# andvg3/LipVQ-VAE

Measured on AMD Instinct MI355X. Metric: actions tokenized/sec (encode+quantize) at B=4096 T=128 K=1024, 1/2/4/8 GPU, higher is better.
Workload: dtype f32

## Files before the change

lipvq-vae_amd/csrc/lipvq_fused.hip:

```cpp
#include <string.h>
#include <atomic>

#include "lipvq_mlp.h"
#include "lipvq_screen.h"

#define FUSED_WAVES 8
#define FUSED_THREADS (FUSED_WAVES * 64)
#define FUSED_HIST_MAX 2048
#define LQ_RING8_TC 1
#define LQ_RING8_NB 3
#define LQ_RING13_NB 3
constexpr int fused_ring_tc(int S) { return (S <= 2) ? 4 : (S <= 4) ? 2 : (S == 8) ? LQ_RING8_TC : 1; }
constexpr int fused_ring_nb(int S) { return (S <= 4) ? 4 : (S == 8) ? LQ_RING8_NB : LQ_RING13_NB; }
#define LQ_COARSE_TC_WIDE 2
constexpr int fused_ring_tc_coarse(int S) { return S == 8 ? LQ_COARSE_TC_WIDE * fused_ring_tc(S) : fused_ring_tc(S); }

struct Gelu2 {
    lq_v2f x, t, u, s;
    __device__ __forceinline__ void stage0(float a, float b) {
        x = (lq_v2f){a, b};
        t = x * x;
        u = lq_fma2(t, lq_bc2(0.11111111111111111111f), lq_bc2(-1.0f));
        s = lq_fma2(lq_bc2(0.00012666420661844313f), u, lq_bc2(-0.00043783686123788357f));
        s = lq_fma2(s, u, lq_bc2(0.0008924771682359278f));
// ... 55 lines not shown
    const float* x;
    const float* packed;
    const unsigned char* packed16;
    const unsigned char* prep;
    const float* cb;
    int64_t* idx;
    float* zq;
    unsigned long long* usage;
    float* ze_out;
    int* amb_count;
    int* amb_list;
    const float* w2q;
    float* pre0;
    float* pre1;
    float* pre2;
    int64_t N;
    int A, D, K;
    float gamma;
    int coarse;
    int inplace;
    int defer_ze;
    int nt_ze;
    int ze_ring;
    int keepz;
};

template <int S, bool FAST, bool TRAIN, int WAVES, bool COARSE = false, bool VQ = false, bool KEEPZ = false>
__device__ __forceinline__ void tokenize_body(const TokArgs& a) {
    static_assert(!(FAST && TRAIN), "training uses the parity arithmetic");
    static_assert(!VQ || !FAST, "the ReLU instance: parity arithmetic");
    static_assert(!KEEPZ || (S <= 4 && !FAST && !TRAIN && !COARSE && !VQ), "z_e kept in registers: the narrow parity instances, decided in place");
    constexpr int THREADS = WAVES * 64;
    constexpr int TCF = COARSE ? fused_ring_tc_coarse(S) : fused_ring_tc(S), NBF = fused_ring_nb(S);
    using RingCfg = ScreenCfg<S, TCF, COARSE>;
    constexpr size_t SLAB_STRIDE = ScreenCfg<S, fused_ring_tc(S), false>::STAGE_BYTES;
    constexpr int T0 = 2, T1 = 4, T2 = (S + 1) / 2;
    constexpr int S1 = 16 * T0, S2 = 16 * T1;
    constexpr bool STREAM2 = !FAST && S >= LQ_STREAM2_MIN_S;
    static_assert(!FAST || (S % 2 == 0 && S <= 8), "fast mode: D in {32, 64, 128}");
    extern __shared__ __attribute__((aligned(16))) unsigned char lds[];
#ifdef LQ_STAMPS
    const long long st_top = __builtin_amdgcn_s_memtime();
    const long long st_top_rt = (long long)__builtin_amdgcn_s_memrealtime();
#endif

    const PackedLayout PL = packed_layout(a.A, 32 * T0, 32 * T1, 16 * S);
    const PrepLayout L = prep_layout(a.K, a.D);
    const int S0 = PL.S0;
    const int S0q = (S0 + 3) / 4;
    const int S0h = (a.A + 15) / 16;
    float* w_P0 = reinterpret_cast<float*>(lds);
    float* w_B0 = w_P0 + (FAST ? T0 * S0h * 256 : T0 * S0q * 256);
    float* w_P1 = w_B0 + 32 * T0;
    float* w_B1 = w_P1 + (FAST ? T1 * (2 * T0) * 256 : T1 * (S1 / 4) * 256);
    float* w_P2 = w_B1 + 32 * T1;
    float* w_B2 = w_P2 + (FAST ? T2 * (2 * T1) * 256 : STREAM2 ? 0 : T2 * (S2 / 4) * 256);
    float* w_mu = w_B2 + 32 * T2;
    unsigned char* stage0 = reinterpret_cast<unsigned char*>(w_mu + 16 * S);
    constexpr size_t RING_OWN = (size_t)NBF * RingCfg::STAGE_BYTES + 1024, RING_FINE = lq_ring_bytes<S, fused_ring_tc(S), NBF>();
    constexpr size_t STAGES_BYTES = RING_OWN > RING_FINE ? RING_OWN : RING_FINE;
    static_assert(STAGES_BYTES >= (size_t)WAVES * LQ_DECIDE_BYTES, "the decision's per-wave transposes live in the stage ring");
    constexpr size_t WSLICE = (STAGES_BYTES >= (size_t)WAVES * 8192) ? 8192 : LQ_DECIDE_BYTES;
    static_assert(LQ_DECIDE_BYTES >= 4096 && WSLICE >= LQ_DECIDE_BYTES, "a slice holds the transposes and four staged KiB");
    static_assert(!KEEPZ || WSLICE >= LQ_DECIDE_BYTES + 64 * S, "KEEPZ: one z_e row behind the decision scratch");
    unsigned* hist = reinterpret_cast<unsigned*>(stage0 + ((STAGES_BYTES + 63) & ~(size_t)63));
    const bool use_hist = a.usage && fused_hist_fits<S, FAST>(a.A, a.K);

    const int tid = threadIdx.x, lane = tid & 63;
    const int wave = __builtin_amdgcn_readfirstlane(tid >> 6);
    const int ln = lane & 31, h = lane >> 5;

    const unsigned* hdr = reinterpret_cast<const unsigned*>(a.prep);
    const unsigned char* tiles = a.prep + (COARSE ? L.o_tiles_hi : L.o_tiles);
    const size_t tile_bytes = COARSE ? L.tile_bytes_hi : L.tile_bytes;
    const int sz = lq_scale_exp(1.0f + __uint_as_float(hdr[4]));
    const float fz = lq_pow2f(sz);
    const float fown = lq_pow2f(sz + (int)hdr[3]);
    const float tiny2 = (float)(16 * S) * lq_pow2f(-10 - 2 * sz);
    const int64_t nblk = (a.N + WAVES * 32 - 1) / (WAVES * 32);
    constexpr int XPF = 8;
    const bool x_pref = !FAST && a.A <= 2 * XPF;
    float xq[XPF];
    constexpr int LANE_W_MIN_S = 8;
    auto load_x = [&](int64_t blk_, float (&out)[XPF]) {
        int64_t r_ = (blk_ * WAVES + wave) * 32 + ln;
        r_ = r_ < a.N ? r_ : a.N - 1;
        const int64_t last = a.N * a.A - 1;
        int h_x = h;
        if constexpr (S >= LANE_W_MIN_S) asm volatile("" : "+v"(h_x));
#pragma unroll
        for (int q = 0; q < XPF; ++q) {
            const int k = 2 * q + h_x;
            int64_t i_ = r_ * a.A + k;
            i_ = i_ < last ? i_ : last;
            const float v = a.x[i_];
            out[q] = (k < a.A) ? v : 0.0f;
        }
    };
    if (x_pref) load_x(blockIdx.x, xq);
    lq_ws_begin(a.amb_count);
    {
        static_assert(32 * T1 <= THREADS && 32 * T2 <= THREADS && 16 * S <= THREADS, "one element per thread");
        const float* mu = reinterpret_cast<const float*>(a.prep + L.o_mu);
        auto bias_src = [&](size_t o, int n) { const int i = tid < n ? tid : n - 1; return a.packed[o + 32 * (i >> 5) + 2 * (i & 15) + ((i >> 4) & 1)]; };
        const float vb0 = bias_src(PL.oB0, 32 * T0), vb1 = bias_src(PL.oB1, 32 * T1), vb2 = bias_src(PL.oB2, 32 * T2);
        const float vmu = mu[tid < 16 * S ? tid : 16 * S - 1];
        if (FAST) {
            const float* src = reinterpret_cast<const float*>(a.packed16);
            const int n0 = T0 * S0h * 256, n1 = T1 * (2 * T0) * 256, n2 = T2 * (2 * T1) * 256;
            auto copy16 = [&](float* dst, const float* from, int nfl) {
                const float4* s4 = reinterpret_cast<const float4*>(from);
                float4* d4 = reinterpret_cast<float4*>(dst);
                const int nv = nfl / 4;
                for (int v0 = tid; v0 < nv; v0 += 4 * THREADS) {
                    float4 r[4];
#pragma unroll
                    for (int q = 0; q < 4; ++q) { const int v = v0 + q * THREADS; r[q] = s4[v < nv ? v : nv - 1]; }
#pragma unroll
                    for (int q = 0; q < 4; ++q) { const int v = v0 + q * THREADS; if (v < nv) d4[v] = r[q]; }
                }
            };
            copy16(w_P0, src, n0);
            copy16(w_P1, src + n0, n1);
            copy16(w_P2, src + n0 + n1, n2);
        } else {
            constexpr int NV1 = T1 * (S1 / 4) * 64, NV2 = STREAM2 ? 0 : T2 * (S2 / 4) * 64;
            constexpr int R1 = (NV1 + THREADS - 1) / THREADS, R2 = (NV2 + THREADS - 1) / THREADS;
            const float* P0 = a.packed + PL.oP0;
            const float* P1 = a.packed + PL.oP1;
            const float* P2 = a.packed + PL.oP2;
            float4 r1[R1], r2[R2 > 0 ? R2 : 1];
#pragma unroll
            for (int it = 0; it < R1; ++it) {
                int v = tid + it * THREADS;
                v = v < NV1 ? v : NV1 - 1;
                const float* src = P1 + ((size_t)(v >> 6) * 4) * 64 + (v & 63);
                r1[it] = make_float4(src[0], src[64], src[128], src[192]);
            }
#pragma unroll
            for (int it = 0; it < R2; ++it) {
                int v = tid + it * THREADS;
                v = v < NV2 ? v : NV2 - 1;
                const float* src = P2 + ((size_t)(v >> 6) * 4) * 64 + (v & 63);
                r2[it] = make_float4(src[0], src[64], src[128], src[192]);
            }
            const int NV0 = T0 * S0q * 64;
            auto p0_entry = [&](int v0, float (&e)[4]) {
                const int l = v0 & 63, sq = (v0 >> 6) % S0q, t = (v0 >> 6) / S0q;
#pragma unroll
                for (int q = 0; q < 4; ++q) {
                    const int s = 4 * sq + q;
                    const float v = P0[((size_t)t * S0 + (s < S0 ? s : S0 - 1)) * 64 + l];
                    e[q] = (s < S0) ? v : 0.0f;
                }
            };
            float e0[4];
            p0_entry(tid < NV0 ? tid : NV0 - 1, e0);
            if (tid < NV0) *reinterpret_cast<float4*>(w_P0 + (size_t)tid * 4) = make_float4(e0[0], e0[1], e0[2], e0[3]);
            for (int v0 = tid + THREADS; v0 < NV0; v0 += THREADS) {
                float e[4];
                p0_entry(v0, e);
                *reinterpret_cast<float4*>(w_P0 + (size_t)v0 * 4) = make_float4(e[0], e[1], e[2], e[3]);
            }
#pragma unroll
            for (int it = 0; it < R1; ++it) {
                const int v = tid + it * THREADS;
                if (v < NV1) *reinterpret_cast<float4*>(w_P1 + (size_t)v * 4) = r1[it];
            }
#pragma unroll
            for (int it = 0; it < R2; ++it) {
                const int v = tid + it * THREADS;
                if (v < NV2) *reinterpret_cast<float4*>(w_P2 + (size_t)v * 4) = r2[it];
            }
        }
        if (tid < 32 * T0) w_B0[tid] = vb0;
        if (tid < 32 * T1) w_B1[tid] = vb1;
        if (tid < 32 * T2) w_B2[tid] = vb2;
        if (tid < 16 * S) w_mu[tid] = vmu;
        if (use_hist)
            for (int i = tid; i < a.K; i += THREADS) hist[i] = 0u;
    }
// ... 60 lines not shown
                acc[r] = zv;
                const float v = zv - w_mu[32 * t + 2 * r + h_w];
                zt[t][r] = v;
                n2 = lq_fma(v, v, n2);
                amax = fmaxf(amax, lq_abs(v));
            }
          } else {
            if constexpr (!FAST) {
                lq_v2f chk = lq_bc2(0.0f);
#pragma unroll
                for (int r = 0; r < 16; r += 2) chk = lq_nonfinite_acc2((lq_v2f){acc[r], acc[r + 1]}, chk);
                if (__builtin_amdgcn_ballot_w64(!(chk.x == 0.0f && chk.y == 0.0f)) != 0ull) {
#pragma unroll
                    for (int r = 0; r < 16; ++r) acc[r] = lq_sigmoid(acc[r]);
                } else {
#pragma unroll
                    for (int r = 0; r < 16; r += 2) {
                        if (2 * t + (r >> 3) >= S) continue;
                        const lq_v2f z2 = lq_sigmoid2_finite((lq_v2f){acc[r], acc[r + 1]});
                        acc[r] = z2.x; acc[r + 1] = z2.y;
                    }
                }
            }
#pragma unroll
            for (int r = 0; r < 16; ++r) {
                if (2 * t + (r >> 3) >= S) continue;
                const float zv = FAST ? __builtin_amdgcn_rcpf(1.0f + __builtin_amdgcn_exp2f(acc[r] * -1.44269504088896341f)) : acc[r];
                acc[r] = zv;
                const float v = zv - w_mu[32 * t + 2 * r + h_w];
                n2 = lq_fma(v, v, n2);
                const float vs = v * fz;
                const _Float16 vh = (_Float16)vs;
                const float rs = vs - (float)vh;
                ah[2 * t + (r >> 3)][r & 7] = vh;
                al[2 * t + (r >> 3)][r & 7] = (_Float16)rs;
                if constexpr (COARSE) a2lo = lq_fma(rs, rs, a2lo);
            }
          }
            if constexpr (KEEPZ) {
                zkeep[t] = acc;
            } else if (a.ze_out) {
                if (DEFER_ZE && a.defer_ze && t == T2 - 1) zdef = acc;
                else store_ze_tile(row, t, acc);
            }
        };

        if constexpr (!FAST) {
            auto gelu_fixup = [&](f32x16& out, const f32x16& pre) {
                float mx = 0.0f;
#pragma unroll
                for (int r = 0; r < 16; r += 2) asm("v_max3_f32 %0, %1, |%2|, |%3|" : "=v"(mx) : "v"(mx), "v"(pre[r]), "v"(pre[r + 1]));
                if (__builtin_amdgcn_ballot_w64(!(mx * mx < 18.0f)) != 0ull) {
#pragma unroll
                    for (int r = 0; r < 16; ++r)
                        if (!(pre[r] * pre[r] < 18.0f)) out[r] = lq_gelu_tail(pre[r]);
                }
            };
            auto bias16 = [&](const float* wb, int t) {
                f32x16 b;
                const float4* p4 = reinterpret_cast<const float4*>(wb + (2 * t + h) * 16);
#pragma unroll
                for (int q = 0; q < 4; ++q) { const float4 v = p4[q]; b[4 * q] = v.x; b[4 * q + 1] = v.y; b[4 * q + 2] = v.z; b[4 * q + 3] = v.w; }
                return b;
            };
            f32x16 h0[T0];
            constexpr int NTRIP = (16 * S + 63) / 64;
            constexpr int GP = (STAGES_BYTES >= (size_t)WAVES * 8192) ? 8 : 4;
            constexpr int NROUND = NTRIP * (8 / GP);
            unsigned char* gstage = stage0 + (size_t)wave * WSLICE;
            const bool gnow = DEFER_GATHER && have_pend && a.zq;
            if (gnow) lq_gather_dma<GP>(gstage, a.cb, pend_k, pend_ok, pend_row0, a.N, a.D, lane, 0, 0);
            {
#pragma unroll
                for (int t = 0; t < T0; ++t) h0[t] = bias16(w_B0, t);
                if (x_pref) {
#pragma unroll
                    for (int sq = 0; sq < XPF / 4; ++sq) {
                        if (sq < S0q) {
                            float4 av[T0];
#pragma unroll
                            for (int t = 0; t < T0; ++t) av[t] = *reinterpret_cast<const float4*>(w_P0 + ((t * S0q + sq) * 64 + lane_w) * 4);
#pragma unroll
                            for (int q = 0; q < 4; ++q) {
                                const float bv = xq[4 * sq + q];
#pragma unroll
                                for (int t = 0; t < T0; ++t) {
                                    const float aq = q == 0 ? av[t].x : q == 1 ? av[t].y : q == 2 ? av[t].z : av[t].w;
                                    h0[t] = __builtin_amdgcn_mfma_f32_32x32x2f32(aq, bv, h0[t], 0, 0, 0);
                                }
                            }
                        }
                    }
                } else {
                    const float* xr = a.x + (size_t)rowc * a.A;
                    for (int sq = 0; sq < S0q; ++sq) {
                        float4 av[T0];
                        float bvv[4];
#pragma unroll
                        for (int t = 0; t < T0; ++t) av[t] = *reinterpret_cast<const float4*>(w_P0 + ((t * S0q + sq) * 64 + lane_w) * 4);
#pragma unroll
                        for (int q = 0; q < 4; ++q) {
                            const int k = 2 * (4 * sq + q) + h;
                            bvv[q] = (k < a.A) ? xr[k] : 0.0f;
                        }
#pragma unroll
                        for (int q = 0; q < 4; ++q)
#pragma unroll
                            for (int t = 0; t < T0; ++t) {
                                const float aq = q == 0 ? av[t].x : q == 1 ? av[t].y : q == 2 ? av[t].z : av[t].w;
                                h0[t] = __builtin_amdgcn_mfma_f32_32x32x2f32(aq, bvv[q], h0[t], 0, 0, 0);
                            }
                    }
                }
#pragma unroll
                for (int t = 0; t < T0; ++t) {
                    const f32x16 pre = h0[t];
                    if constexpr (TRAIN) lq_tile_store16(a.pre0, 32 * T0, row, row < a.N, t, h, pre, 32 * T0, true);
                    if constexpr (VQ) {
#pragma unroll
                        for (int r = 0; r < 16; ++r) h0[t][r] = pre[r] > 0.0f ? pre[r] : 0.0f;
                    } else {
#pragma unroll
                    for (int r = 0; r < 16; r += 2) {
                        const lq_v2f g2 = lq_gelu_poly2((lq_v2f){pre[r], pre[r + 1]});
                        h0[t][r] = g2.x; h0[t][r + 1] = g2.y;
                    }
                    gelu_fixup(h0[t], pre);
                    }
                }
            }
            if (gnow) {
#pragma unroll
                for (int rd = 0; rd < NROUND; ++rd) {
                    lq_wait_vmcnt<0>();
                    lq_gather_flush<GP>(gstage, a.zq, pend_ok, pend_row0, a.N, a.D, lane, rd / (8 / GP), GP * (rd % (8 / GP)));
                    if (rd + 1 < NROUND) {
                        asm volatile("s_waitcnt lgkmcnt(0)" ::: "memory");
                        lq_gather_dma<GP>(gstage, a.cb, pend_k, pend_ok, pend_row0, a.N, a.D, lane, (rd + 1) / (8 / GP),
                                          GP * ((rd + 1) % (8 / GP)));
                    }
                }
            }
            LQ_STAMP(0);
            f32x16 h1[T1];
            f32x16 pend;
            constexpr bool LUMPED = !VQ && !STREAM2;
            constexpr int G1 = S1 / 4, G2 = S2 / 4;
            auto wread = [&](int gidx) {
                if (STREAM2 && gidx >= T1 * G1) gidx = T1 * G1 - 1;
                return (gidx < T1 * G1) ? *reinterpret_cast<const float4*>(w_P1 + (gidx * 64 + lane_w) * 4)
                                        : *reinterpret_cast<const float4*>(w_P2 + ((gidx - T1 * G1) * 64 + lane_w) * 4);
            };
            auto slab_dma = [&](int t_, int buf_) {
                const unsigned char* src = reinterpret_cast<const unsigned char*>(a.w2q) + (size_t)t_ * (G2 * 1024);
                unsigned char* dst = stage0 + (size_t)buf_ * SLAB_STRIDE;
                unsigned lane16 = (unsigned)lane * 16u;
                asm volatile("" : "+v"(lane16));
#pragma unroll
                for (int j = 0; j < G2 * 1024 / 1024 / WAVES; ++j) {
                    const int off = (wave + j * WAVES) * 1024;
                    const unsigned long long gaddr = (unsigned long long)(uintptr_t)(src + off) + lane16;
                    const unsigned ldsaddr = __builtin_amdgcn_readfirstlane((unsigned)(uintptr_t)(dst + off));
                    unsigned m0_keep;
                    asm volatile("s_mov_b32 %0, m0\n\ts_mov_b32 m0, %2\n\ts_nop 0\n\tglobal_load_lds_dwordx4 %1, off\n\ts_mov_b32 m0, %0"
                                 : "=&s"(m0_keep) : "v"(gaddr), "s"(ldsaddr) : "memory");
                }
            };
// ... 104 lines not shown
                f16x8 bx;
#pragma unroll
                for (int j = 0; j < 8; ++j) {
                    const int k = 16 * s2 + 2 * j + h;
                    bx[j] = (_Float16)((k < a.A) ? xr[k] : 0.0f);
                }
#pragma unroll
                for (int t = 0; t < T0; ++t) {
                    const f16x8 av = *reinterpret_cast<const f16x8*>(wh0 + ((size_t)(t * S0h + s2) * 64 + lane) * 8);
                    h0[t] = __builtin_amdgcn_mfma_f32_32x32x16_f16(av, bx, h0[t], 0, 0, 0);
                }
            }
            f16x8 b0[2 * T0];
#pragma unroll
            for (int t = 0; t < T0; ++t)
#pragma unroll
                for (int r = 0; r < 16; ++r) b0[2 * t + (r >> 3)][r & 7] = (_Float16)lq_gelu(h0[t][r]);
            f16x8 b1[2 * T1];
#pragma unroll
            for (int t = 0; t < T1; ++t) {
                f32x16 acc;
#pragma unroll
                for (int r = 0; r < 16; ++r) acc[r] = w_B1[(2 * t + h) * 16 + r];
#pragma unroll
                for (int s2 = 0; s2 < 2 * T0; ++s2) {
                    const f16x8 av = *reinterpret_cast<const f16x8*>(wh1 + ((size_t)(t * (2 * T0) + s2) * 64 + lane) * 8);
                    acc = __builtin_amdgcn_mfma_f32_32x32x16_f16(av, b0[s2], acc, 0, 0, 0);
                }
#pragma unroll
                for (int r = 0; r < 16; ++r) b1[2 * t + (r >> 3)][r & 7] = (_Float16)lq_gelu(acc[r]);
            }
#pragma unroll
            for (int t = 0; t < T2; ++t) {
                f32x16 acc;
#pragma unroll
                for (int r = 0; r < 16; ++r) acc[r] = w_B2[(2 * t + h) * 16 + r];
#pragma unroll
                for (int s2 = 0; s2 < 2 * T1; ++s2) {
                    const f16x8 av = *reinterpret_cast<const f16x8*>(wh2 + ((size_t)(t * (2 * T1) + s2) * 64 + lane) * 8);
                    acc = __builtin_amdgcn_mfma_f32_32x32x16_f16(av, b1[s2], acc, 0, 0, 0);
                }
                finish_tile(t, acc);
            }
        }
        LQ_STAMP(2);
        n2 += __shfl_xor(n2, 32, 64);
        row_n2 = n2;
        row_fz = fz;
        row_fown = fown;
        if constexpr (VQ) {
            amax = fmaxf(amax, __shfl_xor(amax, 32, 64));
            const int szr = lq_scale_exp(amax);
            const float fzr = lq_pow2f(szr);
            row_fz = fzr;
            row_fown = lq_pow2f(szr + (int)hdr[3]);
#pragma unroll
            for (int t = 0; t < T2; ++t)
#pragma unroll
                for (int r = 0; r < 16; ++r) {
                    if (2 * t + (r >> 3) >= S) continue;
                    const float vs = zt[t][r] * fzr;
                    const _Float16 vh = (_Float16)vs;
                    const float rs = vs - (float)vh;
                    ah[2 * t + (r >> 3)][r & 7] = vh;
                    al[2 * t + (r >> 3)][r & 7] = (_Float16)rs;
                    if constexpr (COARSE) a2lo = lq_fma(rs, rs, a2lo);
                }
        }
        if constexpr (COARSE) a2lo += __shfl_xor(a2lo, 32, 64);
        row_a2 = a2lo;
      };
        encode();
        float frow[16];
        if constexpr (VQ) lq_row_factors(row_fown, lane, frow);
        else {
#pragma unroll
            for (int r = 0; r < 16; ++r) frow[r] = fown;
        }
        float m1[16], m2[16];
        int k1[16];
#pragma unroll
        for (int r = 0; r < 16; ++r) { m1[r] = INFINITY; m2[r] = INFINITY; k1[r] = 0; }
        LQ_STAMP(3);
        if (x_pref) load_x(blk + gridDim.x < nblk ? blk + gridDim.x : blk, xq);
        constexpr bool PACKF = S <= 4 || S > 8 || COARSE;
        const float zn = COARSE ? lq_coarse_zn(row_a2, row_n2, row_fz, row_fown, __uint_as_float(hdr[5])) : 0.0f;
        float znr[16];
        if constexpr (COARSE) lq_row_factors(zn, lane, znr);
        else {
#pragma unroll
            for (int r = 0; r < 16; ++r) znr[r] = 0.0f;
        }
        if constexpr (KEEPZ) {
            lq_screen_core<S, THREADS, TCF, NBF, PACKF, COARSE>(ah, al, tiles, L.ntiles, stage0, tid, frow, znr, m1, m2, k1);
        } else {
            const bool have_def = DEFER_ZE && a.defer_ze && a.ze_out != nullptr;
            const bool wave_def = __builtin_amdgcn_ballot_w64((blk * WAVES + wave) * 32 + ln < a.N) != 0ull;
            auto deferred_ze = [&]() { store_ze_tile((blk * WAVES + wave) * 32 + ln, T2 - 1, zdef); };
            lq_screen_core<S, THREADS, TCF, NBF, PACKF, COARSE, 4, decltype(deferred_ze)>(ah, al, tiles, L.ntiles, stage0, tid, frow, znr, m1, m2, k1, have_def, deferred_ze, wave_def);
        }
        LQ_STAMP(4);
        const unsigned keep_mask = PACKF ? ~((1u << lq_pack_bits(L.ntiles)) - 1u) : 0xffffffffu;
        unsigned char* scratch = stage0 + (size_t)wave * WSLICE;
        const int64_t row0 = (blk * WAVES + wave) * 32;
        const int64_t row = row0 + ln;
        int my_k;
        LqDecision dec;
        bool certified = lq_screen_decide<PACKF, COARSE>(m1, m2, k1, scratch, hdr, row_n2, row_fown, a.gamma, a.K, a.D, lane,
                                                         my_k, dec, PACKF ? lq_pow2f(lq_pack_bits(L.ntiles) - 23) : 0.0f, keep_mask,
                                                         zn, tiles, tile_bytes, ScreenCfg<S, TCF, COARSE>::FRAG_BYTES);
        const bool row_sane = VQ || row_n2 >= tiny2;
        certified = certified && row_sane;
        if constexpr (KEEPZ)
            certified = lq_screen_decide_inplace<PACKF, 2 * S, LIPVQ_DIST_NORM, T2>(
                dec, certified, row_sane, my_k, row0, row < a.N, a.amb_count, nullptr, a.cb, a.K, lane, keep_mask, scratch, zkeep);
        else if (!COARSE && a.inplace)
            certified = lq_screen_decide_inplace<PACKF, 2 * S, VQ ? LIPVQ_DIST_SQSUM : LIPVQ_DIST_NORM>(
                dec, certified, row_sane, my_k, row0 - ze_shift, row < a.N, a.amb_count, a.ze_out, a.cb, a.K, lane, keep_mask, scratch);
        else
            lq_screen_emit<PACKF>(dec, certified, row_sane, my_k, row, row < a.N, a.amb_count, a.amb_list, a.N, a.K, lane, keep_mask, scratch);
        if (h == 0 && row < a.N && certified) {
            a.idx[row] = (int64_t)my_k;
            if (use_hist) atomicAdd(&hist[my_k], 1u);
        }
        if (a.usage && !use_hist) lq_usage_add(a.usage, my_k, h == 0 && row < a.N && certified);
        if (DEFER_GATHER) { pend_k = my_k; pend_ok = certified; pend_row0 = row0; }
        else if (a.zq) lq_screen_gather(a.cb, a.zq, my_k, certified, row0, a.N, a.D, lane);
        if (DEFER_GATHER) have_pend = true;
        LQ_STAMP(5);
        LQ_STAMP(6);
    }
    if (DEFER_GATHER && have_pend && a.zq) lq_screen_gather(a.cb, a.zq, pend_k, pend_ok, pend_row0, a.N, a.D, lane);
#ifdef LQ_STAMPS
    if (lane == 0) {
        long long* dbg = LqWorkspace::from_lists(a.amb_list, a.N).stamps() + ((size_t)blockIdx.x * WAVES + wave) * 16;
        for (int i = 0; i < 7; ++i) dbg[i] = st_acc[i];
        dbg[7] = 0;
        dbg[8] = __builtin_amdgcn_s_memtime() - st_begin;
        dbg[9] = st_begin;
        dbg[10] = st_begin - st_top;
        dbg[11] = (long long)__builtin_amdgcn_s_memrealtime();
        dbg[12] = st_top_rt;
    }
#endif
    lq_ws_publish(a.amb_count);
    if (use_hist) {
        for (int i = tid; i < a.K; i += THREADS) {
            const unsigned c = hist[i];
            if (c) atomicAdd(&a.usage[i], (unsigned long long)c);
        }
    }
}

template <int S, bool FAST, bool TRAIN = false, bool COARSE = false, bool VQ = false, bool KEEPZ = false>
__global__ __launch_bounds__(FUSED_THREADS) void tokenize_kernel(TokArgs a) {
    tokenize_body<S, FAST, TRAIN, FUSED_WAVES, COARSE, VQ, KEEPZ>(a);
}
template <int S, bool FAST, bool TRAIN, bool COARSE = false, bool KEEPZ = false>
__global__ __launch_bounds__(256) __attribute__((amdgpu_waves_per_eu(1, 1))) void tokenize_kernel_w4(TokArgs a) {
    tokenize_body<S, FAST, TRAIN, 4, COARSE, false, KEEPZ>(a);
}

__global__ void mlp3_pack_f16_kernel(const float* __restrict__ W0, const float* __restrict__ W1, const float* __restrict__ W2,
                                     _Float16* __restrict__ out, int A, int J0, int J1, int D) {
    const int S0h = (A + 15) / 16, S1h = J0 / 16, S2h = J1 / 16;
    const int T0 = J0 / 32, T1 = J1 / 32, T2 = (D + 31) / 32;
    const size_t n0 = (size_t)T0 * S0h * 512, n1 = (size_t)T1 * S1h * 512, n2 = (size_t)T2 * S2h * 512;
    size_t g = (size_t)blockIdx.x * blockDim.x + threadIdx.x;
    if (g >= n0 + n1 + n2) return;
    const float* W;
    int K, J, Sh;
    size_t e = g;
    if (e < n0) { W = W0; K = A; J = J0; Sh = S0h; }
    else if (e < n0 + n1) { e -= n0; W = W1; K = J0; J = J1; Sh = S1h; }
    else { e -= n0 + n1; W = W2; K = J1; J = D; Sh = S2h; }
    const int j = (int)(e & 7), lane = (int)((e >> 3) & 63);
    const size_t ts = e >> 9;
    const int s = (int)(ts % Sh), t = (int)(ts / Sh);
    const int f = 32 * t + feat_of_tile_row(lane & 31);
    const int k = 16 * s + 2 * j + (lane >> 5);
    out[g] = (_Float16)((f < J && k < K) ? W[(size_t)f * K + k] : 0.0f);
}
// ... 293 lines not shown
```

lipvq-vae_amd/csrc/lipvq_screen.h:

```cpp
#ifndef LIPVQ_SCREEN_H_
#define LIPVQ_SCREEN_H_
#include <hip/hip_fp16.h>

#include <type_traits>

#include "lipvq_common.h"

typedef _Float16 f16x8 __attribute__((ext_vector_type(8)));

#define LIPVQ_SCREEN_GAMMA 3.814697265625e-06f
#define SCREEN_WAVES 8

struct PrepLayout {
    int S, Dpad, Kpad, ntiles;
    size_t o_hdr, o_mu, o_tiles, tile_bytes, total;
    size_t o_tiles_hi, tile_bytes_hi;
};

#define LIPVQ_SCREEN_GAMMA_WIDE 1.52587890625e-05f
#define LQ_SCREEN_NARROW_MAX_S 13

__host__ __device__ static inline int lq_screen_S(int D) {
    const int s = (D + 15) / 16;
    return D <= 0 ? 0 : s <= 2 ? 2 : s <= 4 ? 4 : s <= 8 ? 8 : s <= 13 ? 13 : s <= 16 ? 16 : s <= 24 ? 24 : s <= 32 ? 32 : 0;
// ... 22 lines not shown

__device__ __forceinline__ int lq_scale_exp(float maxabs) {
    const int e = (int)((__float_as_uint(maxabs) >> 23) & 0xff) - 127;
    int k = 13 - e;
    k = k < -60 ? -60 : k;
    k = k > 60 ? 60 : k;
    return (maxabs > 0.0f && maxabs < INFINITY) ? k : 0;
}
__device__ __forceinline__ float lq_pow2f(int k) { return __uint_as_float((unsigned)(k + 127) << 23); }

constexpr int screen_default_tc(int S) { return (S <= 2) ? 8 : (S <= 4) ? 4 : (S <= 8) ? 2 : 1; }

template <int S, int TC_ = screen_default_tc(S), bool COARSE = false>
struct ScreenCfg {
    static constexpr int FRAG_BYTES = COARSE ? S * 1024 : S * 2048;
    static constexpr int TILE_BYTES = FRAG_BYTES + 256;
    static constexpr int TC = TC_;
    static constexpr int STAGE_BYTES = TC * TILE_BYTES;
    static constexpr int STAGE_VEC = STAGE_BYTES / 16;
};

template <int S>
struct StandaloneScreen {
    static constexpr int TC = (S <= 2) ? 4 : (S <= 4) ? 2 : 1;
    static constexpr int NB = (S <= 8) ? 4 : 3;
    static constexpr bool PACK = S <= 4;
};

template <bool PACK>
__device__ __forceinline__ void lq_track_one(float v, int id, unsigned keep_mask, float& m1, float& m2, int& k1) {
    if constexpr (PACK) {
        float key;
        asm("v_and_or_b32 %0, %1, %2, %3" : "=v"(key) : "v"(v), "s"(keep_mask), "v"(id));
        m2 = __builtin_amdgcn_fmed3f(key, m1, m2);
        asm("v_min_f32 %0, %1, %2" : "=v"(m1) : "v"(key), "v"(m1));
    } else {
        const bool lt = v < m1;
        k1 = lt ? id : k1;
        m2 = __builtin_amdgcn_fmed3f(v, m1, m2);
        m1 = lt ? v : m1;
    }
}

__device__ __forceinline__ float lq_coarse_zn(float a2lo, float n2, float fz, float fown, float rho) {
    const float A = lq_sqrt(a2lo), B = lq_sqrt(n2) * fz;
    const float t = lq_fma(rho, lq_fma(3.0f, A, B), A);
    return t * (fown / fz) * 1.0009765625f;
}
template <int LO, int HI, bool PACK = false, bool COARSE = false>
__device__ __forceinline__ void lq_track_part(const f32x16& acc, float e2, float en, const float (&frow)[16], const float (&znr)[16],
                                              int id, unsigned keep_mask, float (&m1)[16], float (&m2)[16], int (&k1)[16]) {
#pragma unroll
    for (int r = LO; r < HI; ++r) {
        const float v = COARSE ? acc[r] : lq_fma(e2, frow[r], acc[r]);
        lq_track_one<PACK>(v, id, keep_mask, m1[r], m2[r], k1[r]);
    }
}

template <int S, bool PACK, bool COARSE = false>
__device__ __forceinline__ void lq_track_after_mfma(int j, const f32x16& acc, float e2, float en, const float (&frow)[16],
                                                    const float (&znr)[16], int id, unsigned keep_mask, float (&m1)[16],
                                                    float (&m2)[16], int (&k1)[16]) {
    constexpr int NM = COARSE ? S : 3 * S;
    const int lo = (16 * j) / NM, hi = (16 * (j + 1)) / NM;
#pragma unroll
    for (int r = 0; r < 16; ++r)
        if (r >= lo && r < hi) {
            const float v = COARSE ? acc[r] : lq_fma(e2, frow[r], acc[r]);
            lq_track_one<PACK>(v, id, keep_mask, m1[r], m2[r], k1[r]);
        }
}

template <int N>
__device__ __forceinline__ void lq_wait_vmcnt() {
    static_assert(N >= 0 && N < 64, "vmcnt immediate");
    asm volatile("s_waitcnt vmcnt(%0)" ::"n"(N) : "memory");
}
template <int S, int TC_, int NB>
constexpr size_t lq_ring_bytes() { return (size_t)NB * ScreenCfg<S, TC_>::STAGE_BYTES + 1024; }

__host__ __device__ static inline int lq_pack_bits(int ntiles) { int b = 1; while ((1 << b) < ntiles) ++b; return b; }

struct LqNoDeferred { __device__ __forceinline__ void operator()() const {} };
template <int S, int NT, int TC_ = screen_default_tc(S), int NB = 4, bool PACK = false, bool COARSE = false, int NDEF = 0,
          typename DEFERRED = LqNoDeferred>
__device__ __forceinline__ void lq_screen_core(const f16x8 (&ah)[S], const f16x8 (&al)[S],
                                               const unsigned char* __restrict__ tiles, int ntiles,
                                               unsigned char* stage0, int tid, const float (&frow)[16], const float (&znr)[16],
                                               float (&m1)[16], float (&m2)[16], int (&k1)[16],
                                               bool have_def = false, DEFERRED deferred = DEFERRED(), bool wave_def = true) {
    using C = ScreenCfg<S, TC_, COARSE>;
    static_assert(NB >= 3 && NB <= 4, "ring of 3 or 4 stage buffers");
    constexpr int NW = NT / 64;
    constexpr int CHUNKS = (C::STAGE_BYTES + 1023) / 1024;
    constexpr int CPW = (CHUNKS + NW - 1) / NW;
    constexpr int PD = NB - 1;
    constexpr int NSTEP = C::TC * S;
    constexpr int MID = (C::TC >= 2) ? (C::TC / 2) * S : S / 2;
    constexpr int FR = 2;
    constexpr int FD = FR - 1;
    constexpr int PERIOD = ((C::TC & 1) || (NSTEP % FR)) ? 2 : 1;
    static_assert(C::STAGE_BYTES >= 1024 && C::STAGE_BYTES % 16 == 0, "stage copies are whole KiB pieces");
    static_assert(NSTEP - FD >= MID, "next-stage fragments are read after the hand-over");
    static_assert(CPW * PD < 64, "vmcnt immediate");
    const int lane = tid & 63, ln = lane & 31;
    const int wave = __builtin_amdgcn_readfirstlane(tid >> 6);
    const int nstage = ntiles / C::TC;
    unsigned char* dummy = stage0 + (size_t)NB * C::STAGE_BYTES;
    typedef __attribute__((address_space(3))) void* lds_ptr_t;
    typedef const __attribute__((address_space(1))) void* glb_ptr_t;
    auto stage_dma = [&](int st, int buf) {
        const bool real = st < nstage;
        const unsigned char* src = tiles + (real ? (size_t)st * C::STAGE_BYTES : (size_t)0);
        unsigned char* dst = stage0 + (size_t)buf * C::STAGE_BYTES;
#pragma unroll
        for (int j = 0; j < CPW; ++j) {
            int chunk = wave + j * NW;
            chunk = chunk < CHUNKS ? chunk : CHUNKS - 1;
            int off = chunk * 1024;
            off = off + 1024 <= C::STAGE_BYTES ? off : C::STAGE_BYTES - 1024;
            unsigned char* d = real ? dst + off : dummy;
            __builtin_amdgcn_global_load_lds((glb_ptr_t)(src + off + lane * 16), (lds_ptr_t)d, 16, 0, 0);
        }
    };
    auto frag = [&](const unsigned char* tb, int s, int hl) {
        return COARSE ? *reinterpret_cast<const f16x8*>(tb + ((size_t)s * 64 + lane) * 16)
                      : *reinterpret_cast<const f16x8*>(tb + (((size_t)s * 2 + hl) * 64 + lane) * 16);
    };
    lq_wg_barrier();
#pragma unroll
    for (int p = 0; p < PD; ++p) stage_dma(p, p);
    static_assert((PD - 1) * CPW + NDEF < 64, "vmcnt immediate");
    const bool count_def = NDEF > 0 && have_def && wave_def;
    if (NDEF > 0 && have_def) deferred();
    if (count_def) {
        lq_wait_vmcnt<(PD - 1) * CPW + NDEF>();
    } else {
        lq_wait_vmcnt<(PD - 1) * CPW>();
    }
    lq_wg_barrier();

    f32x16 accA, accB;
#pragma unroll
    for (int r = 0; r < 16; ++r) accB[r] = INFINITY;
    float e2A = 0.0f, e2B = 0.0f;
    int codeA = 0, codeB = 0;
    const unsigned keep_mask = PACK ? ~((1u << lq_pack_bits(ntiles)) - 1u) : 0xffffffffu;
    f16x8 fh[FR], fl[FR];
    float e2q[2] = {0.0f, 0.0f};
    float enq[2] = {0.0f, 0.0f};
    float enA = 0.0f, enB = 0.0f;
#pragma unroll
    for (int g = 0; g < FD; ++g) {
        fh[g] = frag(stage0, g, 0);
        if constexpr (!COARSE) fl[g] = frag(stage0, g, 1);
    }
    e2q[0] = reinterpret_cast<const float*>(stage0 + C::FRAG_BYTES)[ln];
    if constexpr (COARSE) enq[0] = reinterpret_cast<const float*>(stage0 + C::FRAG_BYTES + 128)[ln];
    static_assert(FD <= S, "prologue reads stay in tile 0");
    int buf = 0;
    auto do_stage = [&](auto POS, int st) {
        constexpr int par = (decltype(POS)::value * C::TC) & 1;
        constexpr int so = (decltype(POS)::value * NSTEP) % FR;
        const unsigned char* sb = stage0 + (size_t)buf * C::STAGE_BYTES;
        int nbuf = buf + 1; nbuf = nbuf == NB ? 0 : nbuf;
        const unsigned char* nsb = stage0 + (size_t)nbuf * C::STAGE_BYTES;
#pragma unroll
        for (int g = 0; g < NSTEP; ++g) {
            const int c = g / S, s = g % S;
            if (g == MID) {
                if (count_def && st == 0) lq_wait_vmcnt<(PD >= 2 ? (PD - 2) * CPW : 0) + (PD >= 2 ? NDEF : 0)>();
                else lq_wait_vmcnt<(PD >= 2 ? (PD - 2) * CPW : 0)>();
                lq_wg_barrier();
                int b = buf + PD; b = b >= NB ? b - NB : b;
                stage_dma(st + PD, b);
            }
            f32x16& acc = (((c + par) & 1) == 0) ? accA : accB;
            const f32x16& prev = (((c + par) & 1) == 0) ? accB : accA;
            const float e2_prev = (((c + par) & 1) == 0) ? e2B : e2A;
            const float en_prev = (((c + par) & 1) == 0) ? enB : enA;
            const int code_prev = (((c + par) & 1) == 0) ? codeB : codeA;
            if (s == 0) {
                const float e2c = e2q[(c + par) & 1];
                const float enc = enq[(c + par) & 1];
#pragma unroll
                for (int r = 0; r < 16; ++r) acc[r] = COARSE ? lq_fma(-znr[r], enc, e2c * frow[r]) : 0.0f;
                int code = PACK ? (st * C::TC + c) : (st * C::TC + c) * 32 + ln;
                if constexpr (PACK) asm volatile("" : "+v"(code));
                if (((c + par) & 1) == 0) { e2A = e2c; enA = enc; codeA = code; } else { e2B = e2c; enB = enc; codeB = code; }
            }
            const f16x8 bh = fh[(g + so) % FR];
            f16x8 bl = bh;
            if constexpr (!COARSE) bl = fl[(g + so) % FR];
            auto read_ahead = [&]() {
                const int g1 = g + FD;
                const unsigned char* base = (g1 < NSTEP) ? sb : nsb;
                const int gg = (g1 < NSTEP) ? g1 : g1 - NSTEP;
                const unsigned char* tb = base + (size_t)(gg / S) * C::TILE_BYTES;
                fh[(g1 + so) % FR] = frag(tb, gg % S, 0);
                if constexpr (!COARSE) fl[(g1 + so) % FR] = frag(tb, gg % S, 1);
                if (gg % S == 0) {
                    e2q[(g1 / S + par) & 1] = reinterpret_cast<const float*>(tb + C::FRAG_BYTES)[ln];
                    if constexpr (COARSE) enq[(g1 / S + par) & 1] = reinterpret_cast<const float*>(tb + C::FRAG_BYTES + 128)[ln];
                }
            };
            __builtin_amdgcn_sched_barrier(0);
            acc = __builtin_amdgcn_mfma_f32_32x32x16_f16(ah[s], bh, acc, 0, 0, 0);
            __builtin_amdgcn_sched_barrier(0);
            read_ahead();
            __builtin_amdgcn_sched_barrier(0);
            lq_track_after_mfma<S, PACK, COARSE>(COARSE ? s : 3 * s + 0, prev, e2_prev, en_prev, frow, znr, code_prev, keep_mask, m1, m2, k1);
            __builtin_amdgcn_sched_barrier(0);
            if constexpr (!COARSE) {
                acc = __builtin_amdgcn_mfma_f32_32x32x16_f16(al[s], bh, acc, 0, 0, 0);
                lq_track_after_mfma<S, PACK>(3 * s + 1, prev, e2_prev, en_prev, frow, znr, code_prev, keep_mask, m1, m2, k1);
                __builtin_amdgcn_sched_barrier(0);
                acc = __builtin_amdgcn_mfma_f32_32x32x16_f16(ah[s], bl, acc, 0, 0, 0);
                lq_track_after_mfma<S, PACK>(3 * s + 2, prev, e2_prev, en_prev, frow, znr, code_prev, keep_mask, m1, m2, k1);
                __builtin_amdgcn_sched_barrier(0);
            }
        }
        buf = nbuf;
    };
    for (int st = 0; st < nstage; st += PERIOD) {
        do_stage(std::integral_constant<int, 0>{}, st);
        if constexpr (PERIOD == 2) do_stage(std::integral_constant<int, 1>{}, st + 1);
    }
    lq_track_part<0, 16, PACK, COARSE>(accB, e2B, enB, frow, znr, codeB, keep_mask, m1, m2, k1);
    lq_wait_vmcnt<0>();
    lq_wg_barrier();
}


__device__ __forceinline__ void lq_row_factors(float fown, int lane, float (&frow)[16]) {
    const int h = lane >> 5;
#pragma unroll
    for (int r = 0; r < 16; ++r) frow[r] = __shfl(fown, (r & 3) + 8 * (r >> 2) + 4 * h, 64);
}

#define LQ_DECIDE_STRIDE 36
#define LQ_DECIDE_BYTES (32 * LQ_DECIDE_STRIDE * 4)

struct LqDecision {
    float vv[16];
    float m2min, best, t0, p;
    bool screen_ok;
};

template <bool PACK = false, bool COARSE = false>
__device__ __forceinline__ bool lq_screen_decide(const float (&m1)[16], const float (&m2)[16], const int (&k1)[16],
                                                 unsigned char* wave_lds ,
                                                 const unsigned* hdr, float n2, float fown, float gamma, int K, int D,
                                                 int lane, int& my_k, LqDecision& dec, float pack_eps = 0.0f,
                                                 unsigned keep_mask = 0xffffffffu, float zn = 0.0f,
// ... 453 lines not shown
```

Measured before the change: 1.362 billion.

## Defer next-block x prefetch into screen prologue and batch x loads for small S

```diff
diff --git a/lipvq-vae_amd/csrc/lipvq_fused.hip b/lipvq-vae_amd/csrc/lipvq_fused.hip
--- a/lipvq-vae_amd/csrc/lipvq_fused.hip
+++ b/lipvq-vae_amd/csrc/lipvq_fused.hip
@@ -161,21 +161,41 @@
     const bool x_pref = !FAST && a.A <= 2 * XPF;
     float xq[XPF];
     constexpr int LANE_W_MIN_S = 8;
+    constexpr bool X_BATCHED = S < LANE_W_MIN_S;
     auto load_x = [&](int64_t blk_, float (&out)[XPF]) {
-        int64_t r_ = (blk_ * WAVES + wave) * 32 + ln;
-        r_ = r_ < a.N ? r_ : a.N - 1;
-        const int64_t last = a.N * a.A - 1;
-        int h_x = h;
-        if constexpr (S >= LANE_W_MIN_S) asm volatile("" : "+v"(h_x));
+        if constexpr (!X_BATCHED) {
+            int64_t r_ = (blk_ * WAVES + wave) * 32 + ln;
+            r_ = r_ < a.N ? r_ : a.N - 1;
+            const int64_t last = a.N * a.A - 1;
+            int h_x = h;
+            asm volatile("" : "+v"(h_x));
+#pragma unroll
+            for (int q = 0; q < XPF; ++q) {
+                const int k = 2 * q + h_x;
+                int64_t i_ = r_ * a.A + k;
+                i_ = i_ < last ? i_ : last;
+                const float v = a.x[i_];
+                out[q] = (k < a.A) ? v : 0.0f;
+            }
+            return;
+        }
+        int64_t row0_ = (blk_ * WAVES + wave) * 32;
+        row0_ = row0_ < a.N ? row0_ : a.N - 1;
+        const int64_t left64 = a.N - 1 - row0_;
+        const int left = left64 < 31 ? (int)left64 : 31;
+        const unsigned char* xb = reinterpret_cast<const unsigned char*>(a.x + row0_ * a.A);
+        const int64_t end64 = ((a.N - row0_) * a.A - 1) * 4;
+        const unsigned end = end64 < (int64_t)(32 * 2 * XPF * 4) ? (unsigned)end64 : 32u * 2 * XPF * 4;
+        const unsigned off0 = (unsigned)((ln < left ? ln : left) * a.A + h) * 4u;
 #pragma unroll
         for (int q = 0; q < XPF; ++q) {
-            const int k = 2 * q + h_x;
-            int64_t i_ = r_ * a.A + k;
-            i_ = i_ < last ? i_ : last;
-            const float v = a.x[i_];
-            out[q] = (k < a.A) ? v : 0.0f;
+            unsigned o = off0 + 8u * q;
+            o = o < end ? o : end;
+            out[q] = *reinterpret_cast<const float*>(xb + o);
         }
     };
+    const int x_kmax = a.A - h;
+    auto x_masked = [&](int i, const float (&v)[XPF]) { return (!X_BATCHED || 2 * i < x_kmax) ? v[i] : 0.0f; };
     if (x_pref) load_x(blockIdx.x, xq);
     lq_ws_begin(a.amb_count);
     {
@@ -402,7 +422,7 @@
                             for (int t = 0; t < T0; ++t) av[t] = *reinterpret_cast<const float4*>(w_P0 + ((t * S0q + sq) * 64 + lane_w) * 4);
 #pragma unroll
                             for (int q = 0; q < 4; ++q) {
-                                const float bv = xq[4 * sq + q];
+                                const float bv = x_masked(4 * sq + q, xq);
 #pragma unroll
                                 for (int t = 0; t < T0; ++t) {
                                     const float aq = q == 0 ? av[t].x : q == 1 ? av[t].y : q == 2 ? av[t].z : av[t].w;
@@ -673,7 +693,9 @@
 #pragma unroll
         for (int r = 0; r < 16; ++r) { m1[r] = INFINITY; m2[r] = INFINITY; k1[r] = 0; }
         LQ_STAMP(3);
-        if (x_pref) load_x(blk + gridDim.x < nblk ? blk + gridDim.x : blk, xq);
+        constexpr bool DEFER_X = S <= 4 && !FAST && !TRAIN && !COARSE && !VQ;
+        const int64_t blk_next = blk + gridDim.x < nblk ? blk + gridDim.x : blk;
+        if (!DEFER_X && x_pref) load_x(blk_next, xq);
         constexpr bool PACKF = S <= 4 || S > 8 || COARSE;
         const float zn = COARSE ? lq_coarse_zn(row_a2, row_n2, row_fz, row_fown, __uint_as_float(hdr[5])) : 0.0f;
         float znr[16];
@@ -683,12 +705,18 @@
             for (int r = 0; r < 16; ++r) znr[r] = 0.0f;
         }
         if constexpr (KEEPZ) {
-            lq_screen_core<S, THREADS, TCF, NBF, PACKF, COARSE>(ah, al, tiles, L.ntiles, stage0, tid, frow, znr, m1, m2, k1);
+            auto deferred_x = [&]() { load_x(blk_next, xq); };
+            lq_screen_core<S, THREADS, TCF, NBF, PACKF, COARSE, 0, decltype(deferred_x), DEFER_X ? XPF : 0>(
+                ah, al, tiles, L.ntiles, stage0, tid, frow, znr, m1, m2, k1, false, deferred_x, true, DEFER_X && x_pref);
         } else {
             const bool have_def = DEFER_ZE && a.defer_ze && a.ze_out != nullptr;
             const bool wave_def = __builtin_amdgcn_ballot_w64((blk * WAVES + wave) * 32 + ln < a.N) != 0ull;
-            auto deferred_ze = [&]() { store_ze_tile((blk * WAVES + wave) * 32 + ln, T2 - 1, zdef); };
-            lq_screen_core<S, THREADS, TCF, NBF, PACKF, COARSE, 4, decltype(deferred_ze)>(ah, al, tiles, L.ntiles, stage0, tid, frow, znr, m1, m2, k1, have_def, deferred_ze, wave_def);
+            auto deferred_ze = [&]() {
+                if (have_def) store_ze_tile((blk * WAVES + wave) * 32 + ln, T2 - 1, zdef);
+                if (DEFER_X && x_pref) load_x(blk_next, xq);
+            };
+            lq_screen_core<S, THREADS, TCF, NBF, PACKF, COARSE, 4, decltype(deferred_ze), DEFER_X ? XPF : 0>(
+                ah, al, tiles, L.ntiles, stage0, tid, frow, znr, m1, m2, k1, have_def, deferred_ze, wave_def, DEFER_X && x_pref);
         }
         LQ_STAMP(4);
         const unsigned keep_mask = PACKF ? ~((1u << lq_pack_bits(L.ntiles)) - 1u) : 0xffffffffu;
diff --git a/lipvq-vae_amd/csrc/lipvq_screen.h b/lipvq-vae_amd/csrc/lipvq_screen.h
--- a/lipvq-vae_amd/csrc/lipvq_screen.h
+++ b/lipvq-vae_amd/csrc/lipvq_screen.h
@@ -128,13 +128,22 @@
 __host__ __device__ static inline int lq_pack_bits(int ntiles) { int b = 1; while ((1 << b) < ntiles) ++b; return b; }
 
 struct LqNoDeferred { __device__ __forceinline__ void operator()() const {} };
+template <int BASE, int NDEF, int NPF>
+__device__ __forceinline__ void lq_wait_vmcnt_deferred(bool cd, bool cp) {
+    static_assert(BASE + NDEF + NPF < 64, "vmcnt immediate");
+    if (NDEF > 0 && NPF > 0 && cd && cp) lq_wait_vmcnt<BASE + NDEF + NPF>();
+    else if (NDEF > 0 && cd) lq_wait_vmcnt<BASE + NDEF>();
+    else if (NPF > 0 && cp) lq_wait_vmcnt<BASE + NPF>();
+    else lq_wait_vmcnt<BASE>();
+}
 template <int S, int NT, int TC_ = screen_default_tc(S), int NB = 4, bool PACK = false, bool COARSE = false, int NDEF = 0,
-          typename DEFERRED = LqNoDeferred>
+          typename DEFERRED = LqNoDeferred, int NPF = 0>
 __device__ __forceinline__ void lq_screen_core(const f16x8 (&ah)[S], const f16x8 (&al)[S],
                                                const unsigned char* __restrict__ tiles, int ntiles,
                                                unsigned char* stage0, int tid, const float (&frow)[16], const float (&znr)[16],
                                                float (&m1)[16], float (&m2)[16], int (&k1)[16],
-                                               bool have_def = false, DEFERRED deferred = DEFERRED(), bool wave_def = true) {
+                                               bool have_def = false, DEFERRED deferred = DEFERRED(), bool wave_def = true,
+                                               bool have_pf = false) {
     using C = ScreenCfg<S, TC_, COARSE>;
     static_assert(NB >= 3 && NB <= 4, "ring of 3 or 4 stage buffers");
     constexpr int NW = NT / 64;
@@ -176,14 +185,11 @@
     lq_wg_barrier();
 #pragma unroll
     for (int p = 0; p < PD; ++p) stage_dma(p, p);
-    static_assert((PD - 1) * CPW + NDEF < 64, "vmcnt immediate");
+    static_assert((PD - 1) * CPW + NDEF + NPF < 64, "vmcnt immediate");
     const bool count_def = NDEF > 0 && have_def && wave_def;
-    if (NDEF > 0 && have_def) deferred();
-    if (count_def) {
-        lq_wait_vmcnt<(PD - 1) * CPW + NDEF>();
-    } else {
-        lq_wait_vmcnt<(PD - 1) * CPW>();
-    }
+    const bool count_pf = NPF > 0 && have_pf;
+    if ((NDEF > 0 && have_def) || count_pf) deferred();
+    lq_wait_vmcnt_deferred<(PD - 1) * CPW, NDEF, NPF>(count_def, count_pf);
     lq_wg_barrier();
 
     f32x16 accA, accB;
@@ -215,7 +221,7 @@
         for (int g = 0; g < NSTEP; ++g) {
             const int c = g / S, s = g % S;
             if (g == MID) {
-                if (count_def && st == 0) lq_wait_vmcnt<(PD >= 2 ? (PD - 2) * CPW : 0) + (PD >= 2 ? NDEF : 0)>();
+                if ((count_def || count_pf) && st == 0) lq_wait_vmcnt_deferred<(PD >= 2 ? (PD - 2) * CPW : 0), (PD >= 2 ? NDEF : 0), (PD >= 2 ? NPF : 0)>(count_def, count_pf);
                 else lq_wait_vmcnt<(PD >= 2 ? (PD - 2) * CPW : 0)>();
                 lq_wg_barrier();
                 int b = buf + PD; b = b >= NB ? b - NB : b;
```

Measured after the change: 1.384 billion (median of 6 runs). 1.7% higher.
